# WeijingShi/Point-GNN

Measured on AMD Instinct MI355X. Metric: KITTI-shaped frames/sec (car_auto_T3 inference: graph build + GNN, 20000 pts/frame, mean E1 602k), higher is better.
Workload: dtype f32

## Files before the change

point-gnn_amd/csrc/gnn.hip:

```cpp
#include <atomic>

#include "mlp_engine.h"
#include "edge_ws.h"
#include "edge_ws_split.h"
#include "pool_ws.h"
#include "pool_split.h"
#include "pool_ws_f16.h"

namespace pgnn {
int g_mlp_blocks_per_cu = 4;
int g_edge_msub = 0;
int g_pool_msub = 0;
int g_mlp_pool_pct = 12;
int g_ws_xcds = 8;
int g_ws_prio = 1;
int g_f16_pool = 1;
int g_b16_force = 0;
int g_ws_pool_pct = 0;
int g_ws_chunk = 2;
int g_ws_balance = 1;
int g_ws_reserve = 0;
void *g_mlp_ts = nullptr;
int g_mlp_debug = 0;
}
// ... 1177 lines not shown
  PGNN_REQUIRE(edges_cap >= 0 && keypoints_cap >= 0 && n_feat >= 0 &&
                   n_feat <= 13 && layers && last_image,
               PGNN_E_INVALID, "pooling_f16x2: bad argument");
  const Dyn de = dyn_of(n_edges), dk = dyn_of(num_keypoints);
  Plan p;
  int rc = make_plan(layers, n_layers, n_feat + 3, p);
  if (rc) return rc;
  const int cus = ws_cus(stream);
  if (!g_f16_pool ||
      !pool_ws_applies(p, g_b16_force ? ((int64_t)1 << 40)
                                      : expected(de, edges_cap), cus))
    return PGNN_E_UNSUPPORTED;
  PGNN_REQUIRE(ld_out >= 16 * 19, PGNN_E_INVALID,
               "pooling_f16x2: ld_out < padded output width");
  if (keypoints_cap == 0) return 0;
  PGNN_REQUIRE(out != nullptr, PGNN_E_INVALID, "pooling_f16x2: null output");
  rc = fill_lowest_rows(out, ld_out, keypoints_cap, dk, stream);
  if (rc) return rc;
  if (edges_cap == 0) return 0;
  PGNN_REQUIRE((n_feat == 0 || point_features) && point_xyz &&
                   keypoint_indices && edges,
               PGNN_E_INVALID, "pooling_f16x2: null input");
  PGNN_REQUIRE((uintptr_t)last_image % 16 == 0 &&
                   (uintptr_t)hidden_image % 16 == 0,
               PGNN_E_INVALID,
               "pooling_f16x2: the images must be 16-byte aligned");
  const PoolArgs pa = {point_features, n_feat, point_xyz, keypoint_indices, edges};
  const SegArgs sa = {out, ld_out, keypoints_cap, edges_sorted & 1};
  PoolWsArgs a = pool_ws_args(p, pa, edges_cap, de.dev, keypoints_cap);
  a.wp = reinterpret_cast<const float *>(last_image);
  a.l2_f16 = g_f16_pool >= 2 ? nullptr : hidden_image;
  rc = pool_ws_out(a, sa, sched_ws, stream);
  if (rc) return rc;
  const size_t lds = (size_t)4 * 19 * 2 * 1024 + 16 * 19 * sizeof(float);
  return launch_lds(a.l2_f16 ? pool_ws_f16x2_kernel<true>
                             : pool_ws_f16x2_kernel<false>,
                    dim3((unsigned)cus), dim3(64 * kWsWaves), lds, stream, a,
                    status);
  PGNN_GUARD_END
}

extern "C" int pgnn_point_set_pooling_fwd(
    const float *point_features, int32_t n_feat, const float *point_xyz,
    const int32_t *keypoint_indices, const int32_t *edges, int64_t n_edges,
    int32_t num_keypoints, const pgnn_fc_layer *layers, int32_t n_layers,
    int32_t edges_sorted, float *out, int64_t ld_out, int32_t *sched_ws,
    void *stream_) {
  PGNN_GUARD_BEGIN
  return pooling_fwd_impl(point_features, n_feat, point_xyz, keypoint_indices,
                          edges, n_edges, num_keypoints, layers, n_layers,
                          edges_sorted, out, ld_out, sched_ws,
                          (hipStream_t)stream_, dyn_of(nullptr),
                          dyn_of(nullptr));
  PGNN_GUARD_END
}

extern "C" int pgnn_point_set_pooling_fwd_dyn(
    const float *point_features, int32_t n_feat, const float *point_xyz,
    const int32_t *keypoint_indices, const int32_t *edges, int64_t edges_cap,
    int32_t keypoints_cap, const pgnn_fc_layer *layers, int32_t n_layers,
    int32_t edges_sorted, float *out, int64_t ld_out, int32_t *sched_ws,
    const pgnn_dyn_count *n_edges, const pgnn_dyn_count *num_keypoints,
    void *stream_) {
  PGNN_GUARD_BEGIN
  PGNN_REQUIRE(n_edges && n_edges->dev && num_keypoints && num_keypoints->dev,
               PGNN_E_INVALID, "pooling_dyn: null count");
  return pooling_fwd_impl(point_features, n_feat, point_xyz, keypoint_indices,
// ... 1148 lines not shown
```

point-gnn_amd/csrc/mlp_engine.h:

```cpp
#pragma once
#include "pgnn_common.h"

namespace pgnn {

#ifndef PGNN_PF4
#define PGNN_PF4 2
#endif
#ifndef PGNN_PF1
#define PGNN_PF1 4
#endif

typedef float v4f __attribute__((ext_vector_type(4)));

struct LayerDev {
  const float *wp;
  int kq;
  int nt;
  int relu_from;
};

struct ChainDev {
  int n;
  LayerDev l[PGNN_MAX_LAYERS];
};
// ... 507 lines not shown
    for (int j = 0; j < TB; ++j) {
      out[t0 + j] = (v4f){0.f, 0.f, 0.f, 0.f};
      w[0][j] = wp[(size_t)(t0 + j) * 64];
    }
#pragma unroll
    for (int q = 0; q < KQ; ++q) {
      if (q + 1 < KQ) {
#pragma unroll
        for (int j = 0; j < TB; ++j)
          w[(q + 1) & 1][j] = wp[((size_t)(q + 1) * NT + t0 + j) * 64];
      }
#pragma unroll
      for (int s = 0; s < 4; ++s)
#pragma unroll
        for (int j = 0; j < TB; ++j)
          out[t0 + j] = __builtin_amdgcn_mfma_f32_16x16x4f32(
              w[q & 1][j][s], in[q][s], out[t0 + j], 0, 0, 0);
      __builtin_amdgcn_sched_barrier(0);
    }
#pragma unroll
    for (int j = 0; j < TB; ++j) {
      const int t = t0 + j;
      const v4f b = *reinterpret_cast<const v4f *>(bias + 16 * t + g4);
#pragma unroll
      for (int r = 0; r < 4; ++r) {
        float v = out[t][r] + b[r];
        if (16 * t + g4 + r >= L.relu_from) v = v > 0.0f ? v : 0.0f;
        out[t][r] = v;
      }
    }
  }
}

template <int KQ, int... NTS>
struct RegChain;

template <int KQ>
struct RegChain<KQ> {
  static __device__ __forceinline__ void run(const ChainDev &, int, int lane,
                                             const v4f (&in)[KQ],
                                             float *__restrict__ rows16,
                                             int ld) {
    float *o = rows16 + (lane & 15) * ld + 4 * (lane >> 4);
#pragma unroll
    for (int q = 0; q < KQ; ++q) *reinterpret_cast<v4f *>(o + 16 * q) = in[q];
  }
};

template <int KQ, int NT, int... REST>
struct RegChain<KQ, NT, REST...> {
  static __device__ __forceinline__ void run(const ChainDev &chain, int li,
                                             int lane, const v4f (&in)[KQ],
                                             float *__restrict__ rows16,
                                             int ld) {
    v4f out[NT];
    reg_layer<KQ, NT>(chain.l[li], lane, in, out);
    RegChain<NT, REST...>::run(chain, li + 1, lane, out, rows16, ld);
  }
};

template <int MSUB, int NT, bool TRANSPOSED, int NW = 4>
__device__ __forceinline__ void layer_pass(const float *in, int ld_in, float *out,
                                           int ld_out, const LayerDev &L, int t0,
                                           int wave, int lane, bool skip_gemm) {
  static_assert(!TRANSPOSED || NW == 4, "transposed stage is 4-wave only");
  v4f acc[MSUB][NT];
// ... 186 lines not shown
```

point-gnn_amd/csrc/pool_split.h:

```cpp
#pragma once
#include "pool_ws.h"

namespace pgnn {

__device__ __forceinline__ void pool_hidden_body(const PoolWsArgs &a,
                                                 const v4f *__restrict__ wl,
                                                 const float *bias_lds,
                                                 int64_t tile_first,
                                                 int64_t tile_last, int lane,
                                                 const int64_t E) {
  constexpr int KQ = 8, NT = 16, NTB = 8;
  if (tile_first >= tile_last) return;
  const int n = lane & 15;
  const int64_t e_first = tile_first * 16;
  const int2 *__restrict__ e2 = reinterpret_cast<const int2 *>(a.edges);
  bool nxt_ok = e_first + n < E;
  int2 nxt = e2[nxt_ok ? e_first + n : 0];
  int nxt_k;
  {
    const int d0 = nxt_ok ? nxt.y : 0;
    nxt_k = a.kp[((unsigned)d0 < (unsigned)a.num_segments) ? d0 : 0];
  }
  for (int64_t tile = tile_first; tile < tile_last; ++tile) {
    const int64_t e0 = tile * 16;
    if (a.prio) __builtin_amdgcn_s_setprio(3);
    int lz;
    asm volatile("v_mov_b32 %0, %1" : "=v"(lz) : "v"(lane));
    const int g = lz >> 4;
    int lz1 = lz + 64 * 64, lz2 = lz + 128 * 64;
    asm volatile("" : "+v"(lz1));
    asm volatile("" : "+v"(lz2));
    const v4f *const wfrag[3] = {wl + lz, wl + lz1, wl + lz2};
    const bool ok = nxt_ok;
    const int my_s = ok ? nxt.x : 0;
    const int my_k = nxt_k;
    nxt_ok = tile + 1 < tile_last && e0 + 16 + n < E;
    nxt = e2[nxt_ok ? e0 + 16 + n : 0];
    v4f x[1];
    x[0] = (v4f){0.f, 0.f, 0.f, 0.f};
    if (ok) {
#pragma unroll
      for (int i = 0; i < 4; ++i) {
        const int c = 4 * g + i;
        float v = 0.0f;
        if (c < a.nfeat) {
          v = a.feat[(int64_t)my_s * a.nfeat + c];
        } else if (c < a.nfeat + 3) {
          const int ax = c - a.nfeat;
          v = a.xyz[3 * (int64_t)my_s + ax] - a.xyz[3 * (int64_t)my_k + ax];
        }
        x[0][i] = v;
      }
    }
    __builtin_amdgcn_sched_barrier(0);
    __builtin_amdgcn_s_setprio(0);
    v4f h1[2], h2[4], h3[KQ];
#ifdef PGNN_POOL_ABL_NO_HIDDEN
#pragma unroll
    for (int q = 0; q < KQ; ++q) h3[q] = x[0];
#else
    reg_layer<1, 2>(a.l0, lane, x, h1);
    reg_layer<2, 4>(a.l1, lane, h1, h2);
    reg_layer<4, 8>(a.l2, lane, h2, h3);
#endif
    __builtin_amdgcn_sched_barrier(0);
    {
      const int dn = nxt_ok ? nxt.y : 0;
      nxt_k = a.kp[((unsigned)dn < (unsigned)a.num_segments) ? dn : 0];
    }
#pragma unroll
    for (int tb = 0; tb < NT; tb += NTB) {
      v4f acc[NTB];
      pool_ws_block<KQ, NT, NTB>(wfrag, tb, h3, acc);
      if (e0 + n < E) {
        float *dstp = a.a4_out + (e0 + n) * a.ld4 + 16 * tb + 4 * g;
#pragma unroll
        for (int t = 0; t < NTB; ++t) {
          const v4f bb =
              *reinterpret_cast<const v4f *>(bias_lds + 16 * (tb + t) + 4 * g);
          v4f y;
#pragma unroll
          for (int r = 0; r < 4; ++r) {
            float xx = acc[t][r] + bb[r];
            if (16 * (tb + t) + 4 * g + r >= a.relu_from)
              xx = xx > 0.0f ? xx : 0.0f;
            y[r] = xx;
          }
          *reinterpret_cast<v4f *>(dstp + 16 * t) = y;
        }
      }
    }
  }
  __builtin_amdgcn_s_setprio(0);
}

#ifndef PGNN_POOLH_WAVES
#define PGNN_POOLH_WAVES 12
#endif
constexpr int kPoolHWaves = PGNN_POOLH_WAVES;
__global__ __launch_bounds__(64 * kPoolHWaves) void pool_hidden_kernel(PoolWsArgs a) {
  constexpr int KQ = 8, NT = 16;
  constexpr int kWsWaves = kPoolHWaves;
  extern __shared__ __attribute__((aligned(16))) char smem[];
  v4f *wl = reinterpret_cast<v4f *>(smem);
  float *bias_lds = reinterpret_cast<float *>(wl + KQ * NT * 64);
  const int lane = threadIdx.x & 63;
  const int wave = __builtin_amdgcn_readfirstlane(threadIdx.x >> 6);
  {
    const v4f *__restrict__ src = reinterpret_cast<const v4f *>(a.wp);
    constexpr int PER = (KQ * NT + kWsWaves - 1) / kWsWaves;
    v4f tmp[PER];
#pragma unroll
    for (int i = 0; i < PER; ++i) {
      const int f = wave + i * kWsWaves;
      tmp[i] = src[(size_t)(f < KQ * NT ? f : 0) * 64 + lane];
    }
    __builtin_amdgcn_sched_barrier(0);
#pragma unroll
    for (int i = 0; i < PER; ++i) {
      const int f = wave + i * kWsWaves;
      if (f < KQ * NT) wl[(size_t)f * 64 + lane] = tmp[i];
    }
    if ((int)threadIdx.x < 16 * NT)
      bias_lds[threadIdx.x] = a.wp[(size_t)KQ * NT * 256 + threadIdx.x];
  }
  __syncthreads();
  int64_t n_edges = a.n_edges;
  if (a.n_dev) {
    const int64_t nd = *a.n_dev;
    n_edges = nd < n_edges ? nd : n_edges;
  }
  const int64_t n_wt = (n_edges + 15) / 16;
  const int xcds = a.slices;
  const int slice = blockIdx.x % xcds, local = blockIdx.x / xcds;
  const int64_t s_first = n_wt * slice / xcds;
  const int64_t s_last = n_wt * (slice + 1) / xcds;
  const int64_t nw = (int64_t)(gridDim.x / xcds) * kWsWaves;
  const int64_t wi = (int64_t)local * kWsWaves + wave;
  const int64_t span = s_last - s_first;
  pool_hidden_body(a, wl, bias_lds, s_first + span * wi / nw,
                   s_first + span * (wi + 1) / nw, lane, n_edges);
}

}
```

point-gnn_amd/csrc/pool_ws.h:

```cpp
#pragma once
#include "edge_ws.h"

namespace pgnn {

struct PoolWsArgs {
  const float *feat;
  int nfeat;
  const float *xyz;
  const int32_t *kp;
  const int32_t *edges;
  int64_t n_edges;
  const int32_t *n_dev;
  LayerDev l0, l1, l2;
  const float *wp;
  int kq, nt;
  int relu_from;
  float *out;
  int64_t ldo;
  int num_segments;
  int sorted;
  int prio;
  long long *ts;
  int32_t *sched;
  int pool_pct;
  int chunk;
  int slices;
  float *a1_out, *a2_out, *a3_out, *a4_out;
  int64_t ld4;
  const void *l2_f16;
};

__device__ __forceinline__ int pool_kp_of(const PoolWsArgs &a, bool ok, int2 e) {
  const int d = ok ? e.y : 0;
  return a.kp[((unsigned)d < (unsigned)a.num_segments) ? d : 0];
}

template <int KQ, int NT, int NTB>
__device__ __forceinline__ void pool_ws_block(const v4f *const (&wfrag)[3],
                                              int tb, const v4f (&h)[KQ],
                                              v4f (&acc)[NTB]) {
  v4f w[2][NTB];
#pragma unroll
  for (int t = 0; t < NTB; ++t) {
    acc[t] = (v4f){0.f, 0.f, 0.f, 0.f};
    w[0][t] = wfrag[(tb + t) >> 6][((tb + t) & 63) * 64];
  }
  __builtin_amdgcn_sched_barrier(0);
#pragma unroll
  for (int q = 0; q < KQ; ++q) {
    __builtin_amdgcn_s_waitcnt(0xC07F);
    __builtin_amdgcn_sched_barrier(0);
    if (q + 1 < KQ) {
#pragma unroll
      for (int t = 0; t < NTB; ++t)
        w[(q + 1) & 1][t] = wfrag[((q + 1) * NT + tb + t) >> 6]
                                 [(((q + 1) * NT + tb + t) & 63) * 64];
    }
#pragma unroll
    for (int s = 0; s < 4; ++s)
#pragma unroll
      for (int t = 0; t < NTB; ++t)
        acc[t] = __builtin_amdgcn_mfma_f32_16x16x4f32(w[q & 1][t][s], h[q][s],
                                                      acc[t], 0, 0, 0);
#if PGNN_WS_SCHED == 2
#pragma unroll
    for (int t = 0; t < NTB; ++t) {
      __builtin_amdgcn_sched_group_barrier(0x8 , 3, 0);
      if (q + 1 < KQ)
        __builtin_amdgcn_sched_group_barrier(0x100 , 1, 0);
    }
    __builtin_amdgcn_sched_group_barrier(0x8 , NTB, 0);
#else
    if (q + 1 < KQ)
      __builtin_amdgcn_sched_group_barrier(0x100 , NTB, 0);
    __builtin_amdgcn_sched_group_barrier(0x8 , 4 * NTB, 0);
#endif
    __builtin_amdgcn_sched_barrier(0);
  }
}

template <bool EMIT, class POL = WsMax>
__device__ __forceinline__ void pool_ws_body(const PoolWsArgs &a,
                                             const v4f *__restrict__ wl,
                                             const float *bias_lds,
                                             int64_t tile_first,
                                             int64_t tile_last, int lane,
                                             long long *tsw, int &stamped,
                                             const int64_t E) {
  constexpr int KQ = 8, NT = 19;
  if (tile_first >= tile_last) return;
  const int n = lane & 15;
  const int64_t e_first = tile_first * 16;
  const int64_t e_end = tile_last * 16 < E ? tile_last * 16 : E;
  const int2 *__restrict__ e2 = reinterpret_cast<const int2 *>(a.edges);
  int cur_d = e_first > 0 ? a.edges[2 * (e_first - 1) + 1] : -1;
  int d_after = e_end < E ? a.edges[2 * e_end + 1] : -1;
  cur_d = __builtin_amdgcn_readfirstlane(cur_d);
  d_after = __builtin_amdgcn_readfirstlane(d_after);
  WsRun run = {cur_d, false, false};
  constexpr float kIdentity = POL::kSum ? 0.0f : kFloatLowest;
  v4f carry0[7], carry1[6], carry2[6];
#pragma unroll
  for (int t = 0; t < 7; ++t) {
    carry0[t] = (v4f){kIdentity, kIdentity, kIdentity, kIdentity};
    if (t < 6) {
      carry1[t] = (v4f){kIdentity, kIdentity, kIdentity, kIdentity};
      carry2[t] = (v4f){kIdentity, kIdentity, kIdentity, kIdentity};
    }
  }
  const float inf = opaque_inf();
  bool nxt_ok = e_first + n < E;
  int2 nxt = e2[nxt_ok ? e_first + n : 0];
  int nxt_k = pool_kp_of(a, nxt_ok, nxt);
  for (int64_t tile = tile_first;; ++tile) {
    const bool fin = tile >= tile_last;
    const int64_t e0 = tile * 16;
    if (a.prio) __builtin_amdgcn_s_setprio(3);
    int lz;
    asm volatile("v_mov_b32 %0, %1" : "=v"(lz) : "v"(lane));
    const int g = lz >> 4;
    int lz1 = lz + 64 * 64, lz2 = lz + 128 * 64;
    asm volatile("" : "+v"(lz1));
    asm volatile("" : "+v"(lz2));
    const v4f *const wfrag[3] = {wl + lz, wl + lz1, wl + lz2};
    long long *tst = nullptr;
    if (tsw && !fin && stamped < kWsStampTiles) tst = tsw + 8 + 4 * stamped++;
    if (tst) {
      __builtin_amdgcn_sched_barrier(0);
      const long long c = __builtin_readcyclecounter();
      if (lane == 0) tst[0] = c;
      __builtin_amdgcn_sched_barrier(0);
    }
    unsigned starts = 1u;
    int my_d = -1;
    v4f h3[KQ];
    if (fin) {
#pragma unroll
      for (int q = 0; q < KQ; ++q) h3[q] = (v4f){0.f, 0.f, 0.f, 0.f};
    } else {
      const bool ok = nxt_ok;
      const int my_s = ok ? nxt.x : 0;
      my_d = ok ? nxt.y : -1;
      const int my_k = nxt_k;
      nxt_ok = tile + 1 < tile_last && e0 + 16 + n < E;
      nxt = e2[nxt_ok ? e0 + 16 + n : 0];
      v4f x[1];
      x[0] = (v4f){0.f, 0.f, 0.f, 0.f};
      if (ok) {
#pragma unroll
        for (int i = 0; i < 4; ++i) {
          const int c = 4 * g + i;
          float v = 0.0f;
          if (c < a.nfeat) {
            v = a.feat[(int64_t)my_s * a.nfeat + c];
          } else if (c < a.nfeat + 3) {
            const int ax = c - a.nfeat;
            v = a.xyz[3 * (int64_t)my_s + ax] - a.xyz[3 * (int64_t)my_k + ax];
          }
          x[0][i] = v;
        }
      }
      __builtin_amdgcn_sched_barrier(0);
      if (tst) {
        const long long c = __builtin_readcyclecounter();
        if (lane == 0) tst[1] = c;
        __builtin_amdgcn_sched_barrier(0);
      }
      __builtin_amdgcn_s_setprio(0);
      v4f h1[2], h2[4];
#ifdef PGNN_POOL_ABL_NO_HIDDEN
#pragma unroll
      for (int q = 0; q < KQ; ++q) h3[q] = x[0];
      h1[0] = h1[1] = x[0];
#pragma unroll
      for (int q = 0; q < 4; ++q) h2[q] = x[0];
#else
      reg_layer<1, 2>(a.l0, lane, x, h1);
      reg_layer<2, 4>(a.l1, lane, h1, h2);
      reg_layer<4, 8>(a.l2, lane, h2, h3);
#endif
      if constexpr (EMIT) {
        if (e0 + n < E) {
          const int64_t row = e0 + n;
#pragma unroll
          for (int q = 0; q < 2; ++q)
            *reinterpret_cast<v4f *>(a.a1_out + row * 32 + 16 * q + 4 * g) = h1[q];
#pragma unroll
          for (int q = 0; q < 4; ++q)
            *reinterpret_cast<v4f *>(a.a2_out + row * 64 + 16 * q + 4 * g) = h2[q];
#pragma unroll
          for (int q = 0; q < 8; ++q)
            *reinterpret_cast<v4f *>(a.a3_out + row * 128 + 16 * q + 4 * g) = h3[q];
        }
      }
      __builtin_amdgcn_sched_barrier(0);
      nxt_k = pool_kp_of(a, nxt_ok, nxt);
      const int up = __shfl_up(my_d, 1);
      const int prev = n == 0 ? run.cur_d : up;
      starts = (unsigned)(__ballot(my_d != prev) & 0xFFFFull);
    }
    const WsRun run0 = run;
#define PGNN_POOL_WS_BLOCK(NTB, TB, CARRY)                                     \
    {                                                                          \
      v4f acc[NTB];                                                            \
      if (!fin) {                                                              \
        pool_ws_block<KQ, NT, NTB>(wfrag, TB, h3, acc);                        \
        if constexpr (EMIT) {     \
          if (e0 + n < E) {                                                    \
            float *dstp = a.a4_out + (e0 + n) * a.ld4 + 16 * (TB) + 4 * g;     \
            _Pragma("unroll")                                                  \
            for (int t = 0; t < NTB; ++t) {                                    \
              const v4f bb = *reinterpret_cast<const v4f *>(                   \
                  bias_lds + 16 * ((TB) + t) + 4 * g);                         \
              v4f y;                                                           \
              _Pragma("unroll")                                                \
              for (int r = 0; r < 4; ++r) {                                    \
                float xx = acc[t][r] + bb[r];                                  \
                if (16 * ((TB) + t) + 4 * g + r >= a.relu_from)                \
                  xx = xx > 0.0f ? xx : 0.0f;                                  \
                y[r] = xx;                                                     \
              }                                                                \
              *reinterpret_cast<v4f *>(dstp + 16 * t) = y;                     \
            }                                                                  \
          }                                                                    \
        }                                                                      \
      } else {       \
        _Pragma("unroll")        \
        for (int t = 0; t < NTB; ++t) acc[t] = (v4f){0.f, 0.f, 0.f, 0.f};      \
      }                                                                        \
      if (a.prio) __builtin_amdgcn_s_setprio(3);                               \
      run = run0;                                                              \
      if constexpr (POL::kSum)                                                 \
        ws_epilogue_sum<NTB>(a, bias_lds + 16 * (TB), TB, lane, acc, CARRY,    \
                             starts, my_d, run, fin, d_after, inf);            \
      else                                                                     \
        ws_epilogue<NTB>(a, bias_lds + 16 * (TB), TB, lane, acc, CARRY,        \
                         starts, my_d, run, fin, d_after, inf);                \
      __builtin_amdgcn_s_setprio(0);                                           \
    }
    PGNN_POOL_WS_BLOCK(7, 0, carry0)
    PGNN_POOL_WS_BLOCK(6, 7, carry1)
    PGNN_POOL_WS_BLOCK(6, 13, carry2)
#undef PGNN_POOL_WS_BLOCK
    if (fin) break;
    if (tst) {
      __builtin_amdgcn_sched_barrier(0);
      const long long c = __builtin_readcyclecounter();
      if (lane == 0) {
        tst[2] = c;
        tst[3] = c;
      }
    }
  }
  __builtin_amdgcn_s_setprio(0);
}

template <bool EMIT = false, class POL = WsMax>
__global__ __launch_bounds__(64 * kWsWaves) void pool_ws_kernel(PoolWsArgs a) {
  constexpr int KQ = 8, NT = 19;
  extern __shared__ __attribute__((aligned(16))) char smem[];
  v4f *wl = reinterpret_cast<v4f *>(smem);
  float *bias_lds = reinterpret_cast<float *>(wl + KQ * NT * 64);
  const int lane = threadIdx.x & 63;
  const int wave = __builtin_amdgcn_readfirstlane(threadIdx.x >> 6);
  ws_stage<(KQ * NT + kWsWaves - 1) / kWsWaves>(
      a, wl, KQ * NT, [](int f) { return (size_t)f; }, (size_t)KQ * NT * 256,
      0, NT, bias_lds, wave, lane);
  __syncthreads();
  const int64_t n_edges = ws_edge_count(a.n_edges, a.n_dev);
  const int64_t n_wt = (n_edges + 15) / 16;
  const int64_t nw = (int64_t)gridDim.x * kWsWaves;
  const int64_t wi = (int64_t)blockIdx.x * kWsWaves + wave;
  const int64_t pool = ws_pool_size(n_wt, a.sched, a.pool_pct, 2, nw);
  const int64_t span = n_wt - pool;
  int64_t tile_first = span * wi / nw;
  int64_t tile_last = span * (wi + 1) / nw;
  long long *tsw = nullptr;
  if (a.ts) {
    tsw = a.ts + wi * kWsStampStride;
    if (lane == 0) {
      tsw[0] = __builtin_readcyclecounter();
      tsw[2] = __builtin_amdgcn_s_memrealtime();
      tsw[4] = tile_last - tile_first;
      tsw[5] = NT;
      tsw[6] = 0;
    }
  }
  int stamped = 0;
  for (;;) {
    pool_ws_body<EMIT, POL>(a, wl, bias_lds, tile_first, tile_last, lane, tsw,
                       stamped, n_edges);
    if (pool == 0) break;
    const int c = ws_pool_claim(&a.sched[2], a.chunk, lane);
    if (c >= pool) break;
    tile_first = span + c;
    tile_last = tile_first + a.chunk < n_wt ? tile_first + a.chunk : n_wt;
  }
  if (tsw && lane == 0) {
    tsw[1] = __builtin_readcyclecounter();
    tsw[3] = __builtin_amdgcn_s_memrealtime();
    tsw[7] = stamped;
  }
  ws_pool_rearm(a.sched, 1, lane);
}

}
```

point-gnn_amd/csrc/pool_ws_f16.h:

```cpp
#pragma once
#include "edge_ws_split.h"
#include "pool_ws.h"

namespace pgnn {

template <int KB>
__device__ __forceinline__ void pool_split_f16(const v4f (&h)[2 * KB],
                                               v4u (&X0)[KB], v4u (&X1)[KB],
                                               u32 &gmax) {
  const v4f zero[2] = {{0.f, 0.f, 0.f, 0.f}, {0.f, 0.f, 0.f, 0.f}};
#pragma unroll
  for (int kb = 0; kb < KB; ++kb) {
    const v4f p[2] = {h[2 * kb], h[2 * kb + 1]};
    split_block_f16(p, zero, X0[kb], X1[kb], gmax);
  }
}

template <int KB, int NT>
__device__ __forceinline__ void reg_layer_f16(const void *img, int relu_from,
                                              int lane, const v4f (&in)[2 * KB],
                                              v4f (&out)[NT], u32 &gmax) {
  constexpr int TB = 4;
  static_assert(NT % TB == 0, "column tiles come in blocks");
  int zero;
// ... 71 lines not shown
#pragma unroll
  for (int kb = 0; kb < 4; ++kb) {
#pragma unroll
    for (int t = 0; t < NTB; ++t) w1[t] = frag(kb, t, 1);
#pragma unroll
    for (int t = 0; t < NTB; ++t) acc[t] = mfma_f16(w0[t], X0[kb], acc[t]);
#pragma unroll
    for (int t = 0; t < NTB; ++t) alo[t] = mfma_f16(w0[t], X1[kb], alo[t]);
    if (kb + 1 < 4) {
#pragma unroll
      for (int t = 0; t < NTB; ++t) w0[t] = frag(kb + 1, t, 0);
    }
#pragma unroll
    for (int t = 0; t < NTB; ++t) alo[t] = mfma_f16(w1[t], X0[kb], alo[t]);
#pragma unroll
    for (int m = 0; m < 3 * NTB; ++m) {
      __builtin_amdgcn_sched_group_barrier(0x8 , 1, 0);
      if (m < NTB || (m >= 2 * NTB && kb + 1 < 4))
        __builtin_amdgcn_sched_group_barrier(0x100 , 1, 0);
    }
    __builtin_amdgcn_sched_barrier(0);
  }
#pragma unroll
  for (int t = 0; t < NTB; ++t)
#pragma unroll
    for (int r = 0; r < 4; ++r)
      acc[t][r] = __builtin_fmaf(alo[t][r], 1.0f / kF16Scale, acc[t][r]);
}

template <bool L2F16>
__device__ __forceinline__ void pool_ws2_body(const PoolWsArgs &a,
                                              const v4u *__restrict__ wl,
                                              const float *bias_lds,
                                              int64_t tile_first,
                                              int64_t tile_last, int lane,
                                              const int64_t E, u32 &gmax) {
  constexpr int NT = 19;
  if (tile_first >= tile_last) return;
  const int n = lane & 15;
  const int64_t e_first = tile_first * 16;
  const int64_t e_end = tile_last * 16 < E ? tile_last * 16 : E;
  const int2 *__restrict__ e2 = reinterpret_cast<const int2 *>(a.edges);
  int cur_d = e_first > 0 ? a.edges[2 * (e_first - 1) + 1] : -1;
  int d_after = e_end < E ? a.edges[2 * e_end + 1] : -1;
  cur_d = __builtin_amdgcn_readfirstlane(cur_d);
  d_after = __builtin_amdgcn_readfirstlane(d_after);
  WsRun run = {cur_d, false, false};
  v4f carry0[7], carry1[6], carry2[6];
#pragma unroll
  for (int t = 0; t < 7; ++t) {
    carry0[t] = (v4f){kFloatLowest, kFloatLowest, kFloatLowest, kFloatLowest};
    if (t < 6) {
      carry1[t] = (v4f){kFloatLowest, kFloatLowest, kFloatLowest, kFloatLowest};
      carry2[t] = (v4f){kFloatLowest, kFloatLowest, kFloatLowest, kFloatLowest};
    }
  }
  const float inf = opaque_inf();
  bool nxt_ok = e_first + n < E;
  int2 nxt = e2[nxt_ok ? e_first + n : 0];
  int nxt_k = pool_kp_of(a, nxt_ok, nxt);
  for (int64_t tile = tile_first;; ++tile) {
    const bool fin = tile >= tile_last;
    const int64_t e0 = tile * 16;
    int lz;
    asm volatile("v_mov_b32 %0, %1" : "=v"(lz) : "v"(lane));
    const int g = lz >> 4;
    int lz1 = lz + 64 * 64, lz2 = lz + 128 * 64;
    asm volatile("" : "+v"(lz1));
    asm volatile("" : "+v"(lz2));
    const v4u *const wfrag[3] = {wl + lz, wl + lz1, wl + lz2};
    unsigned starts = 1u;
    int my_d = -1;
    v4u X0[4], X1[4];
    if (fin) {
#pragma unroll
      for (int kb = 0; kb < 4; ++kb) X0[kb] = X1[kb] = (v4u){0u, 0u, 0u, 0u};
    } else {
      const bool ok = nxt_ok;
      const int my_s = ok ? nxt.x : 0;
      my_d = ok ? nxt.y : -1;
      const int my_k = nxt_k;
      nxt_ok = tile + 1 < tile_last && e0 + 16 + n < E;
      nxt = e2[nxt_ok ? e0 + 16 + n : 0];
      v4f x[1];
      x[0] = (v4f){0.f, 0.f, 0.f, 0.f};
      if (ok) {
#pragma unroll
        for (int i = 0; i < 4; ++i) {
          const int c = 4 * g + i;
          float v = 0.0f;
          if (c < a.nfeat) {
            v = a.feat[(int64_t)my_s * a.nfeat + c];
          } else if (c < a.nfeat + 3) {
            const int ax = c - a.nfeat;
            v = a.xyz[3 * (int64_t)my_s + ax] - a.xyz[3 * (int64_t)my_k + ax];
          }
          x[0][i] = v;
        }
      }
      __builtin_amdgcn_sched_barrier(0);
      v4f h1[2], h2[4], h3[8];
      reg_layer<1, 2>(a.l0, lane, x, h1);
      reg_layer<2, 4>(a.l1, lane, h1, h2);
      if constexpr (L2F16)
        reg_layer_f16<2, 8>(a.l2_f16, a.l2.relu_from, lane, h2, h3, gmax);
      else
        reg_layer<4, 8>(a.l2, lane, h2, h3);
      __builtin_amdgcn_sched_barrier(0);
      pool_split_f16<4>(h3, X0, X1, gmax);
      nxt_k = pool_kp_of(a, nxt_ok, nxt);
      const int prev = __builtin_amdgcn_update_dpp(run.cur_d, my_d,
                                                   0x111 , 0xF, 0xF,
                                                   false);
      starts = (unsigned)(__ballot(my_d != prev) & 0xFFFFull);
    }
    const WsRun run0 = run;
#define PGNN_POOL_WS2_BLOCK(NTB, TB, CARRY)                                    \
    {                                                                          \
      v4f acc[NTB];                                                            \
      if (!fin) {                                                              \
        pool_ws2_block<NT, NTB>(wfrag, TB, X0, X1, acc);                       \
      } else {                                                                 \
        _Pragma("unroll")                                                      \
        for (int t = 0; t < NTB; ++t) acc[t] = (v4f){0.f, 0.f, 0.f, 0.f};      \
      }                                                                        \
      run = run0;                                                              \
      ws_epilogue<NTB>(a, bias_lds + 16 * (TB), TB, lane, acc, CARRY, starts,  \
                       my_d, run, fin, d_after, inf);                          \
    }
    PGNN_POOL_WS2_BLOCK(7, 0, carry0)
    PGNN_POOL_WS2_BLOCK(6, 7, carry1)
    PGNN_POOL_WS2_BLOCK(6, 13, carry2)
#undef PGNN_POOL_WS2_BLOCK
    if (fin) break;
  }
}

template <bool L2F16>
__global__ __launch_bounds__(64 * kWsWaves) void pool_ws_f16x2_kernel(
    PoolWsArgs a, int32_t *status) {
  constexpr int KB = 4, NT = 19;
  extern __shared__ __attribute__((aligned(16))) char smem[];
  v4u *wl = reinterpret_cast<v4u *>(smem);
  float *bias_lds = reinterpret_cast<float *>(wl + KB * NT * 2 * 64);
  const int lane = threadIdx.x & 63;
  const int wave = __builtin_amdgcn_readfirstlane(threadIdx.x >> 6);
  ws_stage<(KB * NT * 2 + kWsWaves - 1) / kWsWaves>(
      a, wl, KB * NT * 2, [](int f) { return (size_t)f; },
      (size_t)KB * NT * 2 * 256, 0, NT, bias_lds, wave, lane);
  __syncthreads();
  const int64_t n_edges = ws_edge_count(a.n_edges, a.n_dev);
  const int64_t n_wt = (n_edges + 15) / 16;
  const int64_t nw = (int64_t)gridDim.x * kWsWaves;
  const int64_t wi = (int64_t)blockIdx.x * kWsWaves + wave;
  const int64_t pool = ws_pool_size(n_wt, a.sched, a.pool_pct, 2, nw);
  const int64_t span = n_wt - pool;
  int64_t tile_first = span * wi / nw;
  int64_t tile_last = span * (wi + 1) / nw;
  u32 gmax = 0;
  for (;;) {
    pool_ws2_body<L2F16>(a, wl, bias_lds, tile_first, tile_last, lane, n_edges,
                         gmax);
    if (pool == 0) break;
    const int c = ws_pool_claim(&a.sched[2], a.chunk, lane);
    if (c >= pool) break;
    tile_first = span + c;
    tile_last = tile_first + a.chunk < n_wt ? tile_first + a.chunk : n_wt;
  }
  if (status && ((gmax & 0xffffu) >= 0x7800u || (gmax >> 16) >= 0x7800u))
    atomicOr(status, 1);
  ws_pool_rearm(a.sched, 1, lane);
}

}
```

point-gnn_amd/csrc/ws_launch.h:

```cpp
#pragma once
#include "ws_partition.h"

namespace {
using namespace pgnn;

inline int ws_cus(int cus) {
  return (g_ws_reserve > 0 && cus - g_ws_reserve >= 64) ? cus - g_ws_reserve : cus;
}
inline int ws_cus(hipStream_t stream) { return ws_cus(stream_cu_count(stream)); }

inline int ws_slices(int cus) { return ws_slice_count(cus, g_ws_xcds); }
inline bool ws_feasible(int nt, int ntmax, int cus) {
  return pgnn::ws_feasible(nt, ntmax, cus, ws_slices(cus));
}

inline int ws_partition_rc(int why) {
  PGNN_REQUIRE(why != kWsTooFewCus, PGNN_E_UNSUPPORTED,
               "edge_ws: too few CUs for the column groups");
  PGNN_REQUIRE(why == kWsOk, PGNN_E_UNSUPPORTED,
               "edge_ws: column tiles do not group");
  return 0;
}

template <int KQ, int NTMAX>
// ... 51 lines not shown
int launch_edge_ws(const LayerDev &L, const EdgeArgs &ea, int64_t n_edges,
                   const SegArgs &sa, int cus, int32_t *sched,
                   hipStream_t stream, float *rows_out = nullptr,
                   int64_t ld_rows = 0, float *h1_out = nullptr,
                   const int32_t *n_dev = nullptr) {
  EdgeWsArgs a;
  const int rc = plan_edge_ws<KQ, NTMAX>(a, L, ea, n_edges, sa, cus, sched,
                                         rows_out, ld_rows, h1_out, n_dev);
  return rc ? rc : run_edge_ws<KQ, NTMAX, false, POL>(a, cus, stream);
}

template <class POL = WsMax>
bool edge_ws_applies(const Plan &p, int64_t n_edges, int cus) {
  if (g_mlp_debug & 2048) return false;
  const LayerDev &L = p.chain.l[0];
  if (p.chain.n != 1 || L.kq != L.nt || (L.nt != 19 && L.nt != 16)) return false;
  if (cus < 64 || cus % 8 != 0) return false;
  if (!ws_feasible(L.nt, L.nt == 19 ? 7 : 8, cus)) return false;
  if ((size_t)L.kq * (L.nt == 19 ? 7 : 8) * 1024 + 16 * 8 * sizeof(float) >
      device_max_lds())
    return false;
  if (g_mlp_debug & 4096) return true;
  return n_edges >= (int64_t)16 * 2 * kWsWaves * cus;
}

template <class POL = WsMax>
bool pool_ws_applies(const Plan &p, int64_t n_edges, int cus) {
  if (g_mlp_debug & (8192 | 1024)) return false;
  const ChainDev &c = p.chain;
  if (c.n != 4 || c.l[0].kq != 1 || c.l[0].nt != 2 || c.l[1].nt != 4 ||
      c.l[2].nt != 8 || c.l[3].kq != 8 || c.l[3].nt != 19)
    return false;
  if (cus < 8) return false;
  if ((size_t)8 * 19 * 1024 + 16 * 19 * sizeof(float) > device_max_lds())
    return false;
  if (g_mlp_debug & 16384) return true;
  return n_edges >= (int64_t)16 * 2 * kWsWaves * cus;
}

PoolWsArgs pool_ws_args(const Plan &p, const PoolArgs &pa, int64_t n_edges,
                        const int32_t *n_dev, int num_segments) {
  PoolWsArgs a = {};
  a.feat = pa.feat;
  a.nfeat = pa.nfeat;
  a.xyz = pa.xyz;
  a.kp = pa.kp;
  a.edges = pa.edges;
  a.n_edges = n_edges;
  a.n_dev = n_dev;
  a.l0 = p.chain.l[0];
  a.l1 = p.chain.l[1];
  a.l2 = p.chain.l[2];
  a.wp = p.chain.l[3].wp;
  a.kq = p.chain.l[3].kq;
  a.nt = p.chain.l[3].nt;
  a.relu_from = p.chain.l[3].relu_from;
  a.num_segments = num_segments;
  return a;
}

int pool_ws_out(PoolWsArgs &a, const SegArgs &sa, int32_t *sched,
                hipStream_t stream) {
  a.out = sa.out;
  a.ldo = sa.ldo;
  a.sorted = sa.sorted;
  a.sched = g_ws_pool_pct > 0 ? sched : nullptr;
  a.pool_pct = g_ws_pool_pct;
  a.chunk = 1;
  PGNN_HIP((hipError_t)arm_sched(a.sched, stream));
  return 0;
}

template <class POL = WsMax>
int launch_pool_ws(const Plan &p, const PoolArgs &pa, int64_t n_edges,
                   const SegArgs &sa, int cus, int32_t *sched,
                   hipStream_t stream, float *const *acts = nullptr,
                   int64_t ld4 = 0, const int32_t *n_dev = nullptr) {
  PoolWsArgs a = pool_ws_args(p, pa, n_edges, n_dev, sa.num_segments);
  if (acts) {
    a.a1_out = acts[0];
    a.a2_out = acts[1];
    a.a3_out = acts[2];
    a.a4_out = acts[3];
    a.ld4 = ld4;
  }
  a.prio = g_ws_prio;
  a.ts = (long long *)g_mlp_ts;
  const int rc = pool_ws_out(a, sa, sched, stream);
  if (rc) return rc;
  const size_t lds = (size_t)8 * 19 * 1024 + 16 * 19 * sizeof(float);
  auto kern = pool_ws_kernel<false, POL>;
  if constexpr (!POL::kSum) {
    if (acts) kern = pool_ws_kernel<true>;
  }
  return launch_lds(kern, dim3((unsigned)cus), dim3(64 * kWsWaves), lds, stream,
                    a);
}

constexpr int kPoolSplitHidden = 256;
bool pool_split_applies(const Plan &p, int64_t n_edges, int cus) {
  if (g_mlp_debug & (8192 | 1024)) return false;
  const ChainDev &c = p.chain;
  if (c.n != 5 || c.l[0].kq != 1 || c.l[0].nt != 2 || c.l[1].nt != 4 ||
      c.l[2].nt != 8 || c.l[3].kq != 8 || c.l[3].nt != 16 || c.l[4].kq != 16 ||
      c.l[4].nt != 32)
    return false;
  if (cus < 64 || cus % 8 != 0) return false;
  if (!ws_feasible(c.l[4].nt, 8, cus)) return false;
  if ((size_t)16 * 8 * 1024 + 16 * 16 * sizeof(float) > device_max_lds())
    return false;
  if (g_mlp_debug & 16384) return true;
  return n_edges >= (int64_t)16 * 2 * kWsWaves * cus;
}

int launch_pool_split(const Plan &p, const PoolArgs &pa, int64_t n_edges,
                      const SegArgs &sa, int cus, int32_t *sched,
                      hipStream_t stream, const int32_t *n_dev, float *hidden) {
  const EdgeArgs ea = {hidden, nullptr, kPoolSplitHidden, pa.edges};
  EdgeWsArgs e;
  int rc = plan_edge_ws<16, 8>(e, p.chain.l[4], ea, n_edges, sa, cus, sched,
                               nullptr, 0, nullptr, n_dev);
  if (rc) return rc;
  PoolWsArgs a = pool_ws_args(p, pa, n_edges, n_dev, sa.num_segments);
  a.prio = g_ws_prio;
  a.a4_out = hidden;
  a.ld4 = kPoolSplitHidden;
  a.slices = 8;
  const size_t lds = (size_t)8 * 16 * 1024 + 16 * 16 * sizeof(float);
  rc = launch_lds(pool_hidden_kernel, dim3((unsigned)cus),
                  dim3(64 * kPoolHWaves), lds, stream, a);
  return rc ? rc : run_edge_ws<16, 8, true>(e, cus, stream);
}

template <class Arith>
struct SplitHost;
template <>
struct SplitHost<Bf16x3> {
  static constexpr const char *kName = "edge_bf16x3";
  static constexpr int kNtMax10 = 5, kNtMax8 = 5;
  static constexpr double kTileCost = 960.0, kRowCost = 2400.0;
  static int prio() { return g_ws_prio; }
};
template <>
struct SplitHost<F16x2> {
  static constexpr const char *kName = "edge_f16x2";
  static constexpr int kNtMax10 = 7, kNtMax8 = 6;
  static constexpr double kTileCost = 480.0, kRowCost = 1600.0;
  static int prio() { return 0; }
};

template <class Arith>
std::string split_msg(const char *what) {
  return std::string(SplitHost<Arith>::kName) + ": " + what;
}

template <class Arith, int KB, int NTMAX>
int launch_edge_ws_split(EdgeWsArgs &a, int nt, int cus, int32_t *status,
                         hipStream_t stream) {
  using H = SplitHost<Arith>;
  const int rc = ws_partition_rc(ws_partition(a, nt, NTMAX, cus, ws_slices(cus)));
  if (rc) return rc;
// ... 78 lines not shown
```

Measured before the change: 326.0.

## Stage small pooling MLP weights in LDS and prefetch rows and weights ahead

Copies layer-0 weights and the biases of the first three pooling MLP layers into LDS when the kernel starts. Layer 0 then reads from LDS, and layers 1 and 2 get their first weight fragments prefetched into registers one layer ahead. The gather of the next tile's point features and xyz is also issued early, overlapping with the current tile's final-layer MFMA blocks. The goal is to hide global-load latency on the hidden-layer chain, at the cost of extra LDS per block, higher register pressure, and added scheduling constraints.

```diff
diff --git a/point-gnn_amd/csrc/gnn.hip b/point-gnn_amd/csrc/gnn.hip
--- a/point-gnn_amd/csrc/gnn.hip
+++ b/point-gnn_amd/csrc/gnn.hip
@@ -1233,7 +1233,8 @@
   a.l2_f16 = g_f16_pool >= 2 ? nullptr : hidden_image;
   rc = pool_ws_out(a, sa, sched_ws, stream);
   if (rc) return rc;
-  const size_t lds = (size_t)4 * 19 * 2 * 1024 + 16 * 19 * sizeof(float);
+  const size_t lds =
+      (size_t)4 * 19 * 2 * 1024 + 16 * 19 * sizeof(float) + kPoolSmallBytes;
   return launch_lds(a.l2_f16 ? pool_ws_f16x2_kernel<true>
                              : pool_ws_f16x2_kernel<false>,
                     dim3((unsigned)cus), dim3(64 * kWsWaves), lds, stream, a,
diff --git a/point-gnn_amd/csrc/mlp_engine.h b/point-gnn_amd/csrc/mlp_engine.h
--- a/point-gnn_amd/csrc/mlp_engine.h
+++ b/point-gnn_amd/csrc/mlp_engine.h
@@ -563,6 +563,138 @@
   }
 }
 
+
+constexpr int kPoolSmallB0 = 0, kPoolSmallB1 = 32, kPoolSmallB2 = 96;
+constexpr int kPoolSmallW0 = 224;
+constexpr int kPoolSmallFloats = kPoolSmallW0 + 2 * 256;
+constexpr size_t kPoolSmallBytes = kPoolSmallFloats * sizeof(float);
+
+struct PoolSmallReq {
+  v4f w;
+  float b;
+};
+__device__ __forceinline__ PoolSmallReq pool_small_request(const float *wp0,
+                                                           const float *wp1,
+                                                           const float *wp2,
+                                                           int tid) {
+  PoolSmallReq r;
+  r.w = reinterpret_cast<const v4f *>(wp0)[tid < 128 ? tid : 127];
+  const int i = tid < kPoolSmallW0 ? tid : kPoolSmallW0 - 1;
+  const float *src = i < kPoolSmallB1   ? wp0 + 1 * 2 * 256 + i
+                     : i < kPoolSmallB2 ? wp1 + 2 * 4 * 256 + (i - kPoolSmallB1)
+                                        : wp2 + 4 * 8 * 256 + (i - kPoolSmallB2);
+  r.b = *src;
+  return r;
+}
+__device__ __forceinline__ void pool_small_write(const PoolSmallReq &r,
+                                                 float *small_lds, int tid) {
+  if (tid < 128) reinterpret_cast<v4f *>(small_lds + kPoolSmallW0)[tid] = r.w;
+  if (tid < kPoolSmallW0) small_lds[tid] = r.b;
+}
+
+template <int NT>
+__device__ __forceinline__ void reg_prefetch_w(const float *wp_, int lane,
+                                               v4f (&w0)[NT]) {
+  int zero;
+  asm volatile("s_mov_b32 %0, 0" : "=s"(zero));
+  const v4f *__restrict__ wp = reinterpret_cast<const v4f *>(wp_) + lane + zero;
+#pragma unroll
+  for (int j = 0; j < NT; ++j) w0[j] = wp[(size_t)j * 64];
+}
+
+template <int NT>
+__device__ __forceinline__ void reg_layer0_lds(const float *small_lds,
+                                               int relu_from, int lane,
+                                               const v4f (&in)[1],
+                                               v4f (&out)[NT]) {
+  int zero;
+  asm volatile("s_mov_b32 %0, 0" : "=s"(zero));
+  const v4f *wp =
+      reinterpret_cast<const v4f *>(small_lds + kPoolSmallW0) + lane + zero;
+  const int g4 = 4 * (lane >> 4) + zero;
+  v4f w[NT], b[NT];
+#pragma unroll
+  for (int j = 0; j < NT; ++j) {
+    out[j] = (v4f){0.f, 0.f, 0.f, 0.f};
+    w[j] = wp[j * 64];
+  }
+#pragma unroll
+  for (int j = 0; j < NT; ++j)
+    b[j] = *reinterpret_cast<const v4f *>(small_lds + kPoolSmallB0 + 16 * j + g4);
+#pragma unroll
+  for (int s = 0; s < 4; ++s)
+#pragma unroll
+    for (int j = 0; j < NT; ++j)
+      out[j] = __builtin_amdgcn_mfma_f32_16x16x4f32(w[j][s], in[0][s], out[j],
+                                                    0, 0, 0);
+  __builtin_amdgcn_sched_group_barrier(0x100 , 2 * NT, 0);
+  __builtin_amdgcn_sched_group_barrier(0x8 , 4 * NT, 0);
+  __builtin_amdgcn_sched_barrier(0);
+#pragma unroll
+  for (int j = 0; j < NT; ++j)
+#pragma unroll
+    for (int r = 0; r < 4; ++r) {
+      float v = out[j][r] + b[j][r];
+      if (16 * j + g4 + r >= relu_from) v = v > 0.0f ? v : 0.0f;
+      out[j][r] = v;
+    }
+}
+
+template <int KQ, int NT, int NTN>
+__device__ __forceinline__ void reg_layer_pre(
+    const LayerDev &L, int lane, const v4f (&in)[KQ], v4f (&out)[NT],
+    const v4f (&w0)[NT], const float *bias_lds, const float *next_wp,
+    v4f (&nw0)[NTN > 0 ? NTN : 1]) {
+  static_assert(NT <= 8, "one block of column tiles");
+  int zero;
+  asm volatile("s_mov_b32 %0, 0" : "=s"(zero));
+  const v4f *__restrict__ wp =
+      reinterpret_cast<const v4f *>(L.wp) + lane + zero;
+  const int g4 = 4 * (lane >> 4) + zero;
+  v4f w[2][NT], b[NT];
+#pragma unroll
+  for (int j = 0; j < NT; ++j) {
+    out[j] = (v4f){0.f, 0.f, 0.f, 0.f};
+    w[0][j] = w0[j];
+  }
+#pragma unroll
+  for (int q = 0; q < KQ; ++q) {
+    if (q + 1 < KQ) {
+#pragma unroll
+      for (int j = 0; j < NT; ++j)
+        w[(q + 1) & 1][j] = wp[((size_t)(q + 1) * NT + j) * 64];
+    } else {
+#pragma unroll
+      for (int j = 0; j < NT; ++j)
+        b[j] = *reinterpret_cast<const v4f *>(bias_lds + 16 * j + g4);
+      if constexpr (NTN > 0) reg_prefetch_w<NTN>(next_wp, lane, nw0);
+    }
+#pragma unroll
+    for (int s = 0; s < 4; ++s)
+#pragma unroll
+      for (int j = 0; j < NT; ++j)
+        out[j] = __builtin_amdgcn_mfma_f32_16x16x4f32(w[q & 1][j][s], in[q][s],
+                                                      out[j], 0, 0, 0);
+    if (q + 1 < KQ) {
+      __builtin_amdgcn_sched_group_barrier(0x20 , NT, 0);
+    } else {
+      if constexpr (NTN > 0)
+        __builtin_amdgcn_sched_group_barrier(0x20 , NTN, 0);
+      __builtin_amdgcn_sched_group_barrier(0x100 , NT, 0);
+    }
+    __builtin_amdgcn_sched_group_barrier(0x8 , 4 * NT, 0);
+    __builtin_amdgcn_sched_barrier(0);
+  }
+#pragma unroll
+  for (int j = 0; j < NT; ++j)
+#pragma unroll
+    for (int r = 0; r < 4; ++r) {
+      float v = out[j][r] + b[j][r];
+      if (16 * j + g4 + r >= L.relu_from) v = v > 0.0f ? v : 0.0f;
+      out[j][r] = v;
+    }
+}
+
 template <int KQ, int... NTS>
 struct RegChain;
 
diff --git a/point-gnn_amd/csrc/pool_split.h b/point-gnn_amd/csrc/pool_split.h
--- a/point-gnn_amd/csrc/pool_split.h
+++ b/point-gnn_amd/csrc/pool_split.h
@@ -6,6 +6,7 @@
 __device__ __forceinline__ void pool_hidden_body(const PoolWsArgs &a,
                                                  const v4f *__restrict__ wl,
                                                  const float *bias_lds,
+                                                 const float *small_lds,
                                                  int64_t tile_first,
                                                  int64_t tile_last, int lane,
                                                  const int64_t E) {
@@ -21,6 +22,8 @@
     const int d0 = nxt_ok ? nxt.y : 0;
     nxt_k = a.kp[((unsigned)d0 < (unsigned)a.num_segments) ? d0 : 0];
   }
+  PoolRowPre row;
+  pool_row_request(a, lane >> 4, nxt_ok ? nxt.x : 0, nxt_k, row);
   for (int64_t tile = tile_first; tile < tile_last; ++tile) {
     const int64_t e0 = tile * 16;
     if (a.prio) __builtin_amdgcn_s_setprio(3);
@@ -32,26 +35,14 @@
     asm volatile("" : "+v"(lz2));
     const v4f *const wfrag[3] = {wl + lz, wl + lz1, wl + lz2};
     const bool ok = nxt_ok;
-    const int my_s = ok ? nxt.x : 0;
-    const int my_k = nxt_k;
+#ifndef PGNN_POOL_ABL_NO_HIDDEN
+    v4f w1[4];
+    reg_prefetch_w<4>(a.l1.wp, lane, w1);
+#endif
+    v4f x[1];
+    x[0] = pool_row_use(a, g, ok, row);
     nxt_ok = tile + 1 < tile_last && e0 + 16 + n < E;
     nxt = e2[nxt_ok ? e0 + 16 + n : 0];
-    v4f x[1];
-    x[0] = (v4f){0.f, 0.f, 0.f, 0.f};
-    if (ok) {
-#pragma unroll
-      for (int i = 0; i < 4; ++i) {
-        const int c = 4 * g + i;
-        float v = 0.0f;
-        if (c < a.nfeat) {
-          v = a.feat[(int64_t)my_s * a.nfeat + c];
-        } else if (c < a.nfeat + 3) {
-          const int ax = c - a.nfeat;
-          v = a.xyz[3 * (int64_t)my_s + ax] - a.xyz[3 * (int64_t)my_k + ax];
-        }
-        x[0][i] = v;
-      }
-    }
     __builtin_amdgcn_sched_barrier(0);
     __builtin_amdgcn_s_setprio(0);
     v4f h1[2], h2[4], h3[KQ];
@@ -59,9 +50,7 @@
 #pragma unroll
     for (int q = 0; q < KQ; ++q) h3[q] = x[0];
 #else
-    reg_layer<1, 2>(a.l0, lane, x, h1);
-    reg_layer<2, 4>(a.l1, lane, h1, h2);
-    reg_layer<4, 8>(a.l2, lane, h2, h3);
+    pool_hidden_layers(a, small_lds, lane, x, w1, h1, h2, h3);
 #endif
     __builtin_amdgcn_sched_barrier(0);
     {
@@ -72,6 +61,7 @@
     for (int tb = 0; tb < NT; tb += NTB) {
       v4f acc[NTB];
       pool_ws_block<KQ, NT, NTB>(wfrag, tb, h3, acc);
+      if (tb == 0) pool_row_request(a, g, nxt_ok ? nxt.x : 0, nxt_k, row);
       if (e0 + n < E) {
         float *dstp = a.a4_out + (e0 + n) * a.ld4 + 16 * tb + 4 * g;
 #pragma unroll
@@ -106,6 +96,9 @@
   float *bias_lds = reinterpret_cast<float *>(wl + KQ * NT * 64);
   const int lane = threadIdx.x & 63;
   const int wave = __builtin_amdgcn_readfirstlane(threadIdx.x >> 6);
+  float *small_lds = bias_lds + 16 * NT;
+  const PoolSmallReq small =
+      pool_small_request(a.l0.wp, a.l1.wp, a.l2.wp, threadIdx.x);
   {
     const v4f *__restrict__ src = reinterpret_cast<const v4f *>(a.wp);
     constexpr int PER = (KQ * NT + kWsWaves - 1) / kWsWaves;
@@ -124,6 +117,7 @@
     if ((int)threadIdx.x < 16 * NT)
       bias_lds[threadIdx.x] = a.wp[(size_t)KQ * NT * 256 + threadIdx.x];
   }
+  pool_small_write(small, small_lds, threadIdx.x);
   __syncthreads();
   int64_t n_edges = a.n_edges;
   if (a.n_dev) {
@@ -138,7 +132,7 @@
   const int64_t nw = (int64_t)(gridDim.x / xcds) * kWsWaves;
   const int64_t wi = (int64_t)local * kWsWaves + wave;
   const int64_t span = s_last - s_first;
-  pool_hidden_body(a, wl, bias_lds, s_first + span * wi / nw,
+  pool_hidden_body(a, wl, bias_lds, small_lds, s_first + span * wi / nw,
                    s_first + span * (wi + 1) / nw, lane, n_edges);
 }
 
diff --git a/point-gnn_amd/csrc/pool_ws.h b/point-gnn_amd/csrc/pool_ws.h
--- a/point-gnn_amd/csrc/pool_ws.h
+++ b/point-gnn_amd/csrc/pool_ws.h
@@ -35,6 +35,60 @@
   return a.kp[((unsigned)d < (unsigned)a.num_segments) ? d : 0];
 }
 
+struct PoolRowPre {
+  float a[4], b[4];
+};
+__device__ __forceinline__ void pool_row_request(const PoolWsArgs &a, int g,
+                                                 int s, int k, PoolRowPre &p) {
+#pragma unroll
+  for (int i = 0; i < 4; ++i) {
+    const int c = 4 * g + i;
+    int ax = c - a.nfeat;
+    ax = ax < 0 ? 0 : (ax > 2 ? 2 : ax);
+    const float *pa = c < a.nfeat ? a.feat + (int64_t)s * a.nfeat + c
+                                  : a.xyz + 3 * (int64_t)s + ax;
+    p.a[i] = *pa;
+    p.b[i] = a.xyz[3 * (int64_t)k + ax];
+  }
+}
+__device__ __forceinline__ v4f pool_row_use(const PoolWsArgs &a, int g, bool ok,
+                                            const PoolRowPre &p) {
+  v4f x;
+#pragma unroll
+  for (int i = 0; i < 4; ++i) {
+    const int c = 4 * g + i;
+    const float v = c < a.nfeat ? p.a[i] : p.a[i] - p.b[i];
+    x[i] = (ok && c < a.nfeat + 3) ? v : 0.0f;
+  }
+  return x;
+}
+
+__device__ __forceinline__ void pool_row_drop(const PoolRowPre &p) {
+#pragma unroll
+  for (int i = 0; i < 4; ++i) asm volatile("" ::"v"(p.a[i]), "v"(p.b[i]));
+}
+
+template <bool L2 = true>
+__device__ __forceinline__ void pool_hidden_layers(const PoolWsArgs &a,
+                                                   const float *small_lds,
+                                                   int lane, const v4f (&x)[1],
+                                                   const v4f (&w1)[4],
+                                                   v4f (&h1)[2], v4f (&h2)[4],
+                                                   v4f (&h3)[8]) {
+  reg_layer0_lds<2>(small_lds, a.l0.relu_from, lane, x, h1);
+  if constexpr (L2) {
+    v4f w2[8], none[1];
+    reg_layer_pre<2, 4, 8>(a.l1, lane, h1, h2, w1, small_lds + kPoolSmallB1,
+                           a.l2.wp, w2);
+    reg_layer_pre<4, 8, 0>(a.l2, lane, h2, h3, w2, small_lds + kPoolSmallB2,
+                           nullptr, none);
+  } else {
+    v4f none[1];
+    reg_layer_pre<2, 4, 0>(a.l1, lane, h1, h2, w1, small_lds + kPoolSmallB1,
+                           nullptr, none);
+  }
+}
+
 template <int KQ, int NT, int NTB>
 __device__ __forceinline__ void pool_ws_block(const v4f *const (&wfrag)[3],
                                               int tb, const v4f (&h)[KQ],
@@ -83,6 +137,7 @@
 __device__ __forceinline__ void pool_ws_body(const PoolWsArgs &a,
                                              const v4f *__restrict__ wl,
                                              const float *bias_lds,
+                                             const float *small_lds,
                                              int64_t tile_first,
                                              int64_t tile_last, int lane,
                                              long long *tsw, int &stamped,
@@ -112,6 +167,8 @@
   bool nxt_ok = e_first + n < E;
   int2 nxt = e2[nxt_ok ? e_first + n : 0];
   int nxt_k = pool_kp_of(a, nxt_ok, nxt);
+  PoolRowPre row;
+  pool_row_request(a, lane >> 4, nxt_ok ? nxt.x : 0, nxt_k, row);
   for (int64_t tile = tile_first;; ++tile) {
     const bool fin = tile >= tile_last;
     const int64_t e0 = tile * 16;
@@ -134,32 +191,22 @@
     unsigned starts = 1u;
     int my_d = -1;
     v4f h3[KQ];
+    const bool ok = nxt_ok;
+    const int2 cur = nxt;
+    nxt_ok = tile + 1 < tile_last && e0 + 16 + n < E;
+    nxt = e2[nxt_ok ? e0 + 16 + n : 0];
     if (fin) {
 #pragma unroll
       for (int q = 0; q < KQ; ++q) h3[q] = (v4f){0.f, 0.f, 0.f, 0.f};
+      pool_row_drop(row);
     } else {
-      const bool ok = nxt_ok;
-      const int my_s = ok ? nxt.x : 0;
-      my_d = ok ? nxt.y : -1;
-      const int my_k = nxt_k;
-      nxt_ok = tile + 1 < tile_last && e0 + 16 + n < E;
-      nxt = e2[nxt_ok ? e0 + 16 + n : 0];
+      my_d = ok ? cur.y : -1;
+#ifndef PGNN_POOL_ABL_NO_HIDDEN
+      v4f w1[4];
+      reg_prefetch_w<4>(a.l1.wp, lane, w1);
+#endif
       v4f x[1];
-      x[0] = (v4f){0.f, 0.f, 0.f, 0.f};
-      if (ok) {
-#pragma unroll
-        for (int i = 0; i < 4; ++i) {
-          const int c = 4 * g + i;
-          float v = 0.0f;
-          if (c < a.nfeat) {
-            v = a.feat[(int64_t)my_s * a.nfeat + c];
-          } else if (c < a.nfeat + 3) {
-            const int ax = c - a.nfeat;
-            v = a.xyz[3 * (int64_t)my_s + ax] - a.xyz[3 * (int64_t)my_k + ax];
-          }
-          x[0][i] = v;
-        }
-      }
+      x[0] = pool_row_use(a, g, ok, row);
       __builtin_amdgcn_sched_barrier(0);
       if (tst) {
         const long long c = __builtin_readcyclecounter();
@@ -175,9 +222,7 @@
 #pragma unroll
       for (int q = 0; q < 4; ++q) h2[q] = x[0];
 #else
-      reg_layer<1, 2>(a.l0, lane, x, h1);
-      reg_layer<2, 4>(a.l1, lane, h1, h2);
-      reg_layer<4, 8>(a.l2, lane, h2, h3);
+      pool_hidden_layers(a, small_lds, lane, x, w1, h1, h2, h3);
 #endif
       if constexpr (EMIT) {
         if (e0 + n < E) {
@@ -194,11 +239,11 @@
         }
       }
       __builtin_amdgcn_sched_barrier(0);
-      nxt_k = pool_kp_of(a, nxt_ok, nxt);
       const int up = __shfl_up(my_d, 1);
       const int prev = n == 0 ? run.cur_d : up;
       starts = (unsigned)(__ballot(my_d != prev) & 0xFFFFull);
     }
+    nxt_k = pool_kp_of(a, nxt_ok, nxt);
     const WsRun run0 = run;
 #define PGNN_POOL_WS_BLOCK(NTB, TB, CARRY)                                     \
     {                                                                          \
@@ -240,6 +285,7 @@
     }
     PGNN_POOL_WS_BLOCK(7, 0, carry0)
     PGNN_POOL_WS_BLOCK(6, 7, carry1)
+    pool_row_request(a, g, nxt_ok ? nxt.x : 0, nxt_k, row);
     PGNN_POOL_WS_BLOCK(6, 13, carry2)
 #undef PGNN_POOL_WS_BLOCK
     if (fin) break;
@@ -261,11 +307,15 @@
   extern __shared__ __attribute__((aligned(16))) char smem[];
   v4f *wl = reinterpret_cast<v4f *>(smem);
   float *bias_lds = reinterpret_cast<float *>(wl + KQ * NT * 64);
+  float *small_lds = bias_lds + 16 * NT;
   const int lane = threadIdx.x & 63;
   const int wave = __builtin_amdgcn_readfirstlane(threadIdx.x >> 6);
+  const PoolSmallReq small =
+      pool_small_request(a.l0.wp, a.l1.wp, a.l2.wp, threadIdx.x);
   ws_stage<(KQ * NT + kWsWaves - 1) / kWsWaves>(
       a, wl, KQ * NT, [](int f) { return (size_t)f; }, (size_t)KQ * NT * 256,
       0, NT, bias_lds, wave, lane);
+  pool_small_write(small, small_lds, threadIdx.x);
   __syncthreads();
   const int64_t n_edges = ws_edge_count(a.n_edges, a.n_dev);
   const int64_t n_wt = (n_edges + 15) / 16;
@@ -288,8 +338,8 @@
   }
   int stamped = 0;
   for (;;) {
-    pool_ws_body<EMIT, POL>(a, wl, bias_lds, tile_first, tile_last, lane, tsw,
-                       stamped, n_edges);
+    pool_ws_body<EMIT, POL>(a, wl, bias_lds, small_lds, tile_first, tile_last,
+                            lane, tsw, stamped, n_edges);
     if (pool == 0) break;
     const int c = ws_pool_claim(&a.sched[2], a.chunk, lane);
     if (c >= pool) break;
diff --git a/point-gnn_amd/csrc/pool_ws_f16.h b/point-gnn_amd/csrc/pool_ws_f16.h
--- a/point-gnn_amd/csrc/pool_ws_f16.h
+++ b/point-gnn_amd/csrc/pool_ws_f16.h
@@ -127,6 +127,7 @@
 __device__ __forceinline__ void pool_ws2_body(const PoolWsArgs &a,
                                               const v4u *__restrict__ wl,
                                               const float *bias_lds,
+                                              const float *small_lds,
                                               int64_t tile_first,
                                               int64_t tile_last, int lane,
                                               const int64_t E, u32 &gmax) {
@@ -175,6 +176,8 @@
       const int my_s = ok ? nxt.x : 0;
       my_d = ok ? nxt.y : -1;
       const int my_k = nxt_k;
+      v4f w1[4];
+      reg_prefetch_w<4>(a.l1.wp, lane, w1);
       nxt_ok = tile + 1 < tile_last && e0 + 16 + n < E;
       nxt = e2[nxt_ok ? e0 + 16 + n : 0];
       v4f x[1];
@@ -195,12 +198,9 @@
       }
       __builtin_amdgcn_sched_barrier(0);
       v4f h1[2], h2[4], h3[8];
-      reg_layer<1, 2>(a.l0, lane, x, h1);
-      reg_layer<2, 4>(a.l1, lane, h1, h2);
+      pool_hidden_layers<!L2F16>(a, small_lds, lane, x, w1, h1, h2, h3);
       if constexpr (L2F16)
         reg_layer_f16<2, 8>(a.l2_f16, a.l2.relu_from, lane, h2, h3, gmax);
-      else
-        reg_layer<4, 8>(a.l2, lane, h2, h3);
       __builtin_amdgcn_sched_barrier(0);
       pool_split_f16<4>(h3, X0, X1, gmax);
       nxt_k = pool_kp_of(a, nxt_ok, nxt);
@@ -238,11 +238,15 @@
   extern __shared__ __attribute__((aligned(16))) char smem[];
   v4u *wl = reinterpret_cast<v4u *>(smem);
   float *bias_lds = reinterpret_cast<float *>(wl + KB * NT * 2 * 64);
+  float *small_lds = bias_lds + 16 * NT;
   const int lane = threadIdx.x & 63;
   const int wave = __builtin_amdgcn_readfirstlane(threadIdx.x >> 6);
+  const PoolSmallReq small =
+      pool_small_request(a.l0.wp, a.l1.wp, a.l2.wp, threadIdx.x);
   ws_stage<(KB * NT * 2 + kWsWaves - 1) / kWsWaves>(
       a, wl, KB * NT * 2, [](int f) { return (size_t)f; },
       (size_t)KB * NT * 2 * 256, 0, NT, bias_lds, wave, lane);
+  pool_small_write(small, small_lds, threadIdx.x);
   __syncthreads();
   const int64_t n_edges = ws_edge_count(a.n_edges, a.n_dev);
   const int64_t n_wt = (n_edges + 15) / 16;
@@ -254,8 +258,8 @@
   int64_t tile_last = span * (wi + 1) / nw;
   u32 gmax = 0;
   for (;;) {
-    pool_ws2_body<L2F16>(a, wl, bias_lds, tile_first, tile_last, lane, n_edges,
-                         gmax);
+    pool_ws2_body<L2F16>(a, wl, bias_lds, small_lds, tile_first, tile_last,
+                         lane, n_edges, gmax);
     if (pool == 0) break;
     const int c = ws_pool_claim(&a.sched[2], a.chunk, lane);
     if (c >= pool) break;
diff --git a/point-gnn_amd/csrc/ws_launch.h b/point-gnn_amd/csrc/ws_launch.h
--- a/point-gnn_amd/csrc/ws_launch.h
+++ b/point-gnn_amd/csrc/ws_launch.h
@@ -107,7 +107,8 @@
       c.l[2].nt != 8 || c.l[3].kq != 8 || c.l[3].nt != 19)
     return false;
   if (cus < 8) return false;
-  if ((size_t)8 * 19 * 1024 + 16 * 19 * sizeof(float) > device_max_lds())
+  if ((size_t)8 * 19 * 1024 + 16 * 19 * sizeof(float) + kPoolSmallBytes >
+      device_max_lds())
     return false;
   if (g_mlp_debug & 16384) return true;
   return n_edges >= (int64_t)16 * 2 * kWsWaves * cus;
@@ -163,7 +164,8 @@
   a.ts = (long long *)g_mlp_ts;
   const int rc = pool_ws_out(a, sa, sched, stream);
   if (rc) return rc;
-  const size_t lds = (size_t)8 * 19 * 1024 + 16 * 19 * sizeof(float);
+  const size_t lds =
+      (size_t)8 * 19 * 1024 + 16 * 19 * sizeof(float) + kPoolSmallBytes;
   auto kern = pool_ws_kernel<false, POL>;
   if constexpr (!POL::kSum) {
     if (acts) kern = pool_ws_kernel<true>;
@@ -182,7 +184,8 @@
     return false;
   if (cus < 64 || cus % 8 != 0) return false;
   if (!ws_feasible(c.l[4].nt, 8, cus)) return false;
-  if ((size_t)16 * 8 * 1024 + 16 * 16 * sizeof(float) > device_max_lds())
+  if ((size_t)16 * 8 * 1024 + 16 * 16 * sizeof(float) + kPoolSmallBytes >
+      device_max_lds())
     return false;
   if (g_mlp_debug & 16384) return true;
   return n_edges >= (int64_t)16 * 2 * kWsWaves * cus;
@@ -201,7 +204,8 @@
   a.a4_out = hidden;
   a.ld4 = kPoolSplitHidden;
   a.slices = 8;
-  const size_t lds = (size_t)8 * 16 * 1024 + 16 * 16 * sizeof(float);
+  const size_t lds =
+      (size_t)8 * 16 * 1024 + 16 * 16 * sizeof(float) + kPoolSmallBytes;
   rc = launch_lds(pool_hidden_kernel, dim3((unsigned)cus),
                   dim3(64 * kPoolHWaves), lds, stream, a);
   return rc ? rc : run_edge_ws<16, 8, true>(e, cus, stream);
```

Result: no change. 325.9 (-0.0%).
